# thourihan/DeepfakeDetection

Measured on AMD Instinct MI355X. Metric: train images/sec @224^2 (EfficientNet-B0), higher is better.
Workload: dtype bf16

## Files before the change

deepfakedetection_amd/_lib.py:

```python

from __future__ import annotations

import ctypes
from ctypes import POINTER, Structure, c_double, c_float, c_int, c_int64, c_long, c_size_t, c_uint32, c_void_p
from pathlib import Path

import os as _os

LIB_PATH = Path(_os.environ.get("DFD_LIB_PATH") or Path(__file__).resolve().parent / "libdfd_hip.so")

DFD_OK = 0
ERRORS = {-1: "DFD_EINVAL", -2: "DFD_EUNSUPPORTED", -3: "DFD_ELAUNCH", -4: "DFD_EWORKSPACE"}
F32, BF16 = 0, 1
ACT_NONE, ACT_SILU, ACT_RELU, ACT_GELU = 0, 1, 2, 3
PRO_NONE, PRO_BN_ACT, PRO_BN_ACT_GATE, PRO_AFFINE2 = 0, 1, 2, 3
MAX_PARTIALS = 1024
ADAMW_TABLE_COLS = 5
ADAMW_HP_LEN = 8


class DwShape(Structure):
    _fields_ = [(n, c_int) for n in ("N", "H", "W", "C", "Ho", "Wo", "k", "stride", "pad_top", "pad_left")]


# ... 34 lines not shown
    "dfd_act_bn_bwd_se": (c_int, [c_int, P, P, P, P, P, c_int, P, c_int, c_int, c_int, P, c_int, _PI, P, P, c_int, P, P, P, P, c_int, P]),
    "dfd_prep_weights_multi": (c_int, [P, c_int, P]),
    "dfd_resize_crop_u8": (c_int, [P, P, P, c_int, c_int, c_int, c_int, P]),
    "dfd_augment_u8": (c_int, [P, P, P, c_int, c_int, c_int, P]),
    "dfd_image_prep": (c_int, [P, P, c_int, c_int, c_int, POINTER(c_float), POINTER(c_float), P, P, P]),
    "dfd_pool_ws": (c_size_t, [c_int, c_int, c_int, c_int]),
    "dfd_pool_act": (c_int, [c_int, P, P, c_int, P, c_int, c_int, c_int, P, c_size_t, P]),
    "dfd_pool_bwd_reduce": (c_int, [c_int, P, P, P, c_int, P, c_int, c_int, c_int, P, c_size_t, P]),
    "dfd_scale_rows": (c_int, [c_int, P, P, P, c_int, c_int, c_int, P]),
    "dfd_se_fc_fwd": (c_int, [P, P, P, P, P, c_int, c_int, c_int, c_int, P, P, P, P]),
    "dfd_se_fc_bwd": (c_int, [P, P, P, P, P, P, c_int, c_int, c_int, c_int, P, P, P, P, P, c_int, P, P]),
    "dfd_dwconv_fwd": (c_int, [c_int, P, P, c_int, P, P, POINTER(DwShape), P, c_int, _PI, P]),
    "dfd_dwconv_bwd_data": (c_int, [c_int, P, P, P, P, P, P, c_int, P, POINTER(DwShape), P, c_int, _PI, P]),
    "dfd_dwconv_bwd_weight": (c_int, [c_int, P, P, P, P, P, c_int, P, POINTER(DwShape), c_int, P, c_size_t, P]),
    "dfd_dwconv_bwd_weight_ws": (c_size_t, [POINTER(DwShape)]),
    "dfd_dwconv_bwd_fused": (c_int, [c_int, P, P, P, P, P, P, c_int, P, P, POINTER(DwShape), P, c_int, _PI, c_int, P, c_size_t, P]),
    "dfd_pwconv_fwd": (c_int, [c_int, P, POINTER(Prologue), P, P, P, c_int, c_int, c_int, P, c_int, _PI, P]),
    "dfd_pwconv_wgrad": (c_int, [c_int, P, POINTER(Prologue), c_int, P, POINTER(Prologue), c_int, c_int, P, c_int, P, c_size_t, P]),
    "dfd_pwconv_wgrad_ws": (c_size_t, [c_int, c_int, c_int]),
    "dfd_gradcam_map": (c_int, [P, P, c_int, c_int, c_int, c_int, P, P]),
    "dfd_cam_render": (c_int, [P, c_int, c_int, c_int, c_int, c_int, P, P, P, c_double, P, P, P, c_size_t, P]),
    "dfd_cam_render_ws": (c_size_t, [c_int, c_int, c_int, c_int, c_int]),
    "dfd_pwconv_bwd_fused": (c_int, [c_int, P, P, P, P, P, P, c_int, c_int, c_int, P, P, c_int, P, c_size_t, P]),
    "dfd_pw_prep_weights": (c_int, [c_int, P, P, P, c_int, c_int, P]),
    "dfd_stem_conv_fwd": (c_int, [c_int, P, P, P, POINTER(StemShape), P, c_int, _PI, P]),
    "dfd_stem_conv_wgrad": (c_int, [c_int, P, P, P, P, P, POINTER(StemShape), c_int, P, c_size_t, P]),
    "dfd_stem_conv_wgrad_ws": (c_size_t, [POINTER(StemShape)]),
    "dfd_dropout": (c_int, [P, P, c_float, P, c_int, P]),
    "dfd_linear_fwd": (c_int, [P, P, P, P, c_int, c_int, c_int, P]),
    "dfd_linear_bwd": (c_int, [P, P, P, P, P, P, c_int, c_int, c_int, c_int, P]),
    "dfd_ce_loss": (c_int, [P, P, c_int, c_int, c_float, c_float, P, P, P, P]),
    "dfd_softmax_argmax": (c_int, [P, c_int, c_int, P, P, P]),
    "dfd_adamw_step": (c_int, [P, c_int, P, P]),
    "dfd_bn_eval_coeffs_multi": (c_int, [P, c_int, P]),
    "dfd_sum_batch_begin": (c_int, []),
    "dfd_sum_batch_end": (c_int, []),
    "dfd_sum_batch_end_deferred": (c_int, []),
    "dfd_sum_passengers_flush": (c_int, [P]),
    "dfd_sum_passengers_discard": (c_int, []),
    "dfd_se_fwd": (c_int, [c_int, P, P, c_int, c_int, c_int, c_int, P, P, P, P, c_int, c_int, P, P, P, P, P, c_size_t, P]),
    "dfd_se_bwd": (c_int, [c_int, P, P, P, c_int, c_int, c_int, c_int, P, P, P, P, P, c_int, c_int, P, P, P, P, P, P, c_int,
                           P, c_size_t, P, P]),
    "dfd_pwconv_fwd_eval": (c_int, [c_int, P, P, P, c_int, P, c_int, c_int, c_int, P]),
    "dfd_dwconv_fwd_eval_tiles": (c_int, [c_int, P]),
    "dfd_dwconv_fwd_eval": (c_int, [c_int, P, P, P, c_int, P, P, P, P, P]),
    "dfd_se_fwd_parts": (c_int, [P, c_int, c_int, c_int, c_int, P, P, P, P, c_int, c_int, P, P, P, P, P]),
# ... 122 lines not shown
```

deepfakedetection_amd/csrc/dfd_pwtnw.hip:

```cpp
#include "dfd_pw.h"

#define TNW_MIN_ROWS 16

template <int ROWS, int NA, int NBT, int PA, int PB, int ACT, int DG = 0>
__global__ void __launch_bounds__(DFD_THREADS, NBT > 9 ? 1 : 2)
k_pw_tnw(const bf16* __restrict__ a, ProArgs pa, int Na, const bf16* __restrict__ b, ProArgs pb, int Nb, int M,
         int rows_per_block, int swap, float* __restrict__ ws, const bf16* __restrict__ w_kn = nullptr,
         const bf16* __restrict__ res = nullptr, bf16* __restrict__ dx = nullptr, int wstride = 0, int woff = 0) {
    constexpr int ITA = (ROWS * NA * 2 + 63) / 64;
    constexpr int ITB = (ROWS * NBT * 2 + 63) / 64;
    extern __shared__ __attribute__((aligned(16))) unsigned char smem[];
    const int t = threadIdx.x, lane = t & 63, wave = t >> 6;
    unsigned char* at = smem + wave * (2 * ROWS * 256);
    unsigned char* bt = at + ROWS * 256;
    float* cl = reinterpret_cast<float*>(smem + 4 * 2 * ROWS * 256);
    const bf16* a2 = reinterpret_cast<const bf16*>(pa.a2);
    const bf16* b2 = reinterpret_cast<const bf16*>(pb.a2);
    const int ca = Na >> 3, cb = Nb >> 3;
    float* gc = cl + 3 * (Na + Nb) + wave * 2 * Nb;
    int gimg = -1;

    for (int i = t; i < 3 * Na; i += DFD_THREADS) cl[i] = (PA != DFD_PRO_NONE) ? pa.coef[i] : 0.f;
    for (int i = t; i < 3 * Nb; i += DFD_THREADS) {
        float v = 0.f;
        if (PB == DFD_PRO_AFFINE2) v = pb.coef[i];
        else if (PB != DFD_PRO_NONE && i < 2 * Nb) v = pb.coef[i];
        cl[3 * Na + i] = v;
    }
    for (int i = t; i < 4 * 2 * ROWS * 256 / 16; i += DFD_THREADS) reinterpret_cast<uint4*>(smem)[i] = make_uint4(0, 0, 0, 0);
    if constexpr (DG) {
        const int chunks = wstride >> 4;
        for (int i = t; i < NA * 16 * chunks; i += DFD_THREADS) {
            const int r = i / chunks, c = i - r * chunks;
            uint4 v = make_uint4(0, 0, 0, 0);
            if (r < Na && c < cb) v = *reinterpret_cast<const uint4*>(w_kn + (long)r * Nb + c * 8);
            *reinterpret_cast<uint4*>(smem + woff + r * wstride + c * 16) = v;
        }
    }
    __syncthreads();

    int ra[ITA], cha[ITA], rb[ITB], chb[ITB];
#pragma unroll
    for (int i = 0; i < ITA; ++i) {
        const int idx = lane + 64 * i;
        const bool ok = idx < ROWS * ca;
        ra[i] = ok ? idx / ca : -1;
        cha[i] = ok ? idx - ra[i] * ca : 0;
    }
#pragma unroll
    for (int i = 0; i < ITB; ++i) {
        const int idx = lane + 64 * i;
        const bool ok = idx < ROWS * cb;
        rb[i] = ok ? idx / cb : -1;
        chb[i] = ok ? idx - rb[i] * cb : 0;
    }

    f32x4_t acc[NA][NBT];
#pragma unroll
    for (int x = 0; x < NA; ++x)
#pragma unroll
        for (int y = 0; y < NBT; ++y) acc[x][y] = (f32x4_t){0.f, 0.f, 0.f, 0.f};
    const int na = (Na + 15) >> 4, nbt = (Nb + 15) >> 4;
    constexpr int RT = ROWS / 16;
    f32x4_t accd[DG ? NA : 1][RT];

    const int rows_per_wave = rows_per_block / 4;
    const int mbeg = blockIdx.x * rows_per_block + wave * rows_per_wave;
    int mend = mbeg + rows_per_wave;
    if (mend > M) mend = M;

    uint4 va[ITA], va2[ITA], vb[ITB], vb2[ITB];
    auto load_a = [&](int i, int m0) {
        int row = m0 + (ra[i] < 0 ? 0 : ra[i]);
        row = row < M ? row : M - 1;
        const long off = (long)row * Na + cha[i] * 8;
        va[i] = *reinterpret_cast<const uint4*>(a + off);
        if constexpr (PA == DFD_PRO_AFFINE2) va2[i] = *reinterpret_cast<const uint4*>(a2 + off);
    };
    auto load_b = [&](int i, int m0) {
        int row = m0 + (rb[i] < 0 ? 0 : rb[i]);
        row = row < M ? row : M - 1;
        const long off = (long)row * Nb + chb[i] * 8;
        vb[i] = *reinterpret_cast<const uint4*>(b + off);
        if constexpr (PB == DFD_PRO_AFFINE2) vb2[i] = *reinterpret_cast<const uint4*>(b2 + off);
    };
    auto g_load = [&](int m0) {
#pragma unroll
        for (int i = 0; i < ITA; ++i) load_a(i, m0);
#pragma unroll
        for (int i = 0; i < ITB; ++i) load_b(i, m0);
    };
    auto pro_item = [&](auto mode_tag, uint4 q, uint4 q2, const float* cf, int N, int ch, int m, const ProArgs& pr) -> uint4 {
        constexpr int MODE = decltype(mode_tag)::value;
        if constexpr (MODE == DFD_PRO_NONE) {
            return q;
        } else {
            float v[8], c0[8], c1[8];
            q_to_f(q, v);
            load_f32<8>(cf + ch * 8, c0);
            load_f32<8>(cf + N + ch * 8, c1);
            if constexpr (MODE == DFD_PRO_AFFINE2) {
                float v2[8], c2[8];
                q_to_f(q2, v2);
                load_f32<8>(cf + 2 * N + ch * 8, c2);
#pragma unroll
                for (int j = 0; j < 8; ++j) v[j] = fmaf(c0[j], v[j], fmaf(c1[j], v2[j], c2[j]));
            } else if constexpr (MODE == DFD_PRO_BN_ACT) {
// ... 5 lines not shown
#pragma unroll
                for (int j = 0; j < 8; ++j) v[j] = round_to<bf16>(v[j]) * gt[j];
            }
            return f_to_q(v);
        }
    };
    auto s_store_a = [&](int m0) {
#pragma unroll
        for (int i = 0; i < ITA; ++i) {
            if (ra[i] >= 0) {
                uint4 v = make_uint4(0, 0, 0, 0);
                if (m0 + ra[i] < mend) v = pro_item(std::integral_constant<int, PA>{}, va[i], va2[i], cl, Na, cha[i], m0 + ra[i], pa);
                *reinterpret_cast<uint4*>(at + tn_off_bf16(ra[i], cha[i])) = v;
            }
            load_a(i, m0 + ROWS);
        }
    };
    auto s_store_b = [&](int m0, int grp, auto refill_tag) {
        constexpr bool refill = decltype(refill_tag)::value;
#pragma unroll
        for (int i = 0; i < ITB; ++i) {
            if (rb[i] >= 0 && (chb[i] >> 4) == grp) {
                uint4 v = make_uint4(0, 0, 0, 0);
                if (m0 + rb[i] < mend)
                    v = pro_item(std::integral_constant<int, PB>{}, vb[i], vb2[i], cl + 3 * Na, Nb, chb[i], m0 + rb[i], pb);
                *reinterpret_cast<uint4*>(bt + tn_off_bf16(rb[i], chb[i] & 15)) = v;
            }
            if constexpr (refill) load_b(i, m0 + ROWS);
        }
    };
    auto wave_sync = [&]() {
        __builtin_amdgcn_fence(__ATOMIC_RELEASE, "wavefront");
        __builtin_amdgcn_wave_barrier();
        __builtin_amdgcn_fence(__ATOMIC_ACQUIRE, "wavefront");
    };
    const int g = lane >> 4, li = lane & 15, qrow = li >> 2, pcol = li & 3;
    auto frag = [&](const unsigned char* tile, int ch0) -> short8_t {
        const int ch = ch0 + (pcol >> 1), sub = (pcol & 1) << 3;
        if constexpr (ROWS == 32) {
            const int m_lo = 8 * g + qrow, m_hi = m_lo + 4;
            const short4_t lo = __builtin_amdgcn_ds_read_tr16_b64_v4i16(
                (__attribute__((address_space(3))) short4_t*)(tile + tn_off_bf16(m_lo, ch) + sub));
            const short4_t hi = __builtin_amdgcn_ds_read_tr16_b64_v4i16(
                (__attribute__((address_space(3))) short4_t*)(tile + tn_off_bf16(m_hi, ch) + sub));
            return (short8_t){lo[0], lo[1], lo[2], lo[3], hi[0], hi[1], hi[2], hi[3]};
        } else {
            const short4_t lo = __builtin_amdgcn_ds_read_tr16_b64_v4i16(
                (__attribute__((address_space(3))) short4_t*)(tile + tn_off_bf16(4 * g + qrow, ch) + sub));
            return (short8_t){lo[0], lo[1], lo[2], lo[3], 0, 0, 0, 0};
        }
    };
    auto mma = [&](const short8_t& fx, const short8_t& fy, f32x4_t c) -> f32x4_t {
        if constexpr (ROWS == 32) {
            return __builtin_amdgcn_mfma_f32_16x16x32_bf16(__builtin_bit_cast(bf16x8_t, fx), __builtin_bit_cast(bf16x8_t, fy), c, 0, 0, 0);
        } else {
            const short4_t x4 = (short4_t){fx[0], fx[1], fx[2], fx[3]}, y4 = (short4_t){fy[0], fy[1], fy[2], fy[3]};
            return __builtin_amdgcn_mfma_f32_16x16x16bf16_1k(x4, y4, c, 0, 0, 0);
        }
    };

    constexpr int NGRP = NBT > 8 ? 2 : 1;
    if (mbeg < mend) g_load(mbeg);
    for (int m0 = mbeg; m0 < mend; m0 += ROWS) {
        short8_t fa[NA];
        if constexpr (PB == DFD_PRO_BN_ACT_GATE) {
            const int img0 = pro_image(pb, m0);
            if (img0 != gimg) {
                gimg = img0;
                for (int i = lane; i < 2 * Nb; i += 64) {
                    const int im = img0 + (i >= Nb ? 1 : 0);
                    gc[i] = ((long)im * pb.HW < M) ? pb.gate[(long)im * Nb + (i >= Nb ? i - Nb : i)] : 0.f;
                }
                wave_sync();
            }
        }
        if constexpr (DG) {
#pragma unroll
            for (int x = 0; x < NA; ++x)
#pragma unroll
                for (int j = 0; j < RT; ++j) accd[x][j] = (f32x4_t){0.f, 0.f, 0.f, 0.f};
        }
        s_store_a(m0);
        s_store_b(m0, 0, std::integral_constant<bool, NGRP == 1>{});
        wave_sync();
#pragma unroll
        for (int x = 0; x < NA; ++x)
            if (x < na) fa[x] = frag(at, 2 * x);
#pragma unroll
        for (int grp = 0; grp < NGRP; ++grp) {
            if (grp > 0) {
                wave_sync();
                s_store_b(m0, grp, std::true_type{});
                wave_sync();
            }
#pragma unroll
            for (int y = 0; y < NBT; ++y) {
                if ((y >> 3) != grp || y >= nbt) continue;
                const short8_t fb = frag(bt, 2 * (y & 7));
#pragma unroll
                for (int x = 0; x < NA; ++x)
                    if (x < na)
                        acc[x][y] = mma(fa[x], fb, acc[x][y]);
            }
            if constexpr (DG) {
#pragma unroll
                for (int ks = 0; ks < 4; ++ks) {
                    if (grp * 8 + 2 * ks >= NBT || grp * 8 + 2 * ks >= nbt) continue;
                    const int chl = 4 * ks + g, chg = grp * 16 + chl;
                    uint4 fd[RT];
#pragma unroll
                    for (int j = 0; j < RT; ++j) {
                        fd[j] = *reinterpret_cast<const uint4*>(bt + tn_off_bf16(j * 16 + li, chl));
                        if (chg >= cb) fd[j] = make_uint4(0, 0, 0, 0);
                    }
// ... 86 lines not shown
    hipLaunchKernelGGL((k_pw_tnw<ROWS, NA, NBT, PAV, PBV, ACTV>), dim3(nblocks), dim3(DFD_THREADS), lds, st, (const bf16*)a, pa, \
                       Na, (const bf16*)b, pb, Nb, M, rpb, swap, ws)
    if (mb == DFD_PRO_BN_ACT_GATE) {
        if (act != DFD_ACT_SILU) return DFD_EUNSUPPORTED;
        if (ma == DFD_PRO_AFFINE2) LAUNCH_TNW(DFD_PRO_AFFINE2, DFD_PRO_BN_ACT_GATE, DFD_ACT_SILU);
        else LAUNCH_TNW(DFD_PRO_NONE, DFD_PRO_BN_ACT_GATE, DFD_ACT_SILU);
    } else if (mb == DFD_PRO_BN_ACT) {
        if (ma != DFD_PRO_AFFINE2) return DFD_EUNSUPPORTED;
        if (act == DFD_ACT_GELU) LAUNCH_TNW(DFD_PRO_AFFINE2, DFD_PRO_BN_ACT, DFD_ACT_GELU);
        else if (act == DFD_ACT_SILU) LAUNCH_TNW(DFD_PRO_AFFINE2, DFD_PRO_BN_ACT, DFD_ACT_SILU);
        else return DFD_EUNSUPPORTED;
    } else if (mb == DFD_PRO_AFFINE2) {
        if (ma == DFD_PRO_AFFINE2) return DFD_EUNSUPPORTED;
        LAUNCH_TNW(DFD_PRO_NONE, DFD_PRO_AFFINE2, DFD_ACT_NONE);
    } else {
        if (ma == DFD_PRO_AFFINE2) LAUNCH_TNW(DFD_PRO_AFFINE2, DFD_PRO_NONE, DFD_ACT_NONE);
        else LAUNCH_TNW(DFD_PRO_NONE, DFD_PRO_NONE, DFD_ACT_NONE);
    }
#undef LAUNCH_TNW
    if (hipGetLastError() != hipSuccess) return DFD_ELAUNCH;
    return dfd_launch_sum_partials(ws, nblocks, (long)Na * Nb, dw, accumulate, st);
}

template <int ROWS, int NA, int NBT>
static int tnw_dg_launch(const void* x, int Cin, const void* dz, const dfd_prologue* pro_d, int Cm, const void* w_kn, const void* residual,
                         int M, void* dx, float* dw, int accumulate, float* ws, size_t ws_bytes, hipStream_t st) {
    const ProArgs pa = pro_args(nullptr), pb = pro_args(pro_d);
    int nblocks = NBT > 9 ? 256 : 512;
    int rpb = (M + nblocks - 1) / nblocks;
    rpb = (rpb + 4 * ROWS - 1) / (4 * ROWS) * (4 * ROWS);
    nblocks = (M + rpb - 1) / rpb;
    if ((size_t)(nblocks + nblocks / 32 + 2) * Cin * Cm * 4 > ws_bytes) return DFD_EUNSUPPORTED;
    const int wstride = (Cm + 31) / 32 * 64 + 16;
    int woff = 4 * 2 * ROWS * 256 + 3 * (Cin + Cm) * 4;
    woff = (woff + 15) / 16 * 16;
    const int lds = woff + NA * 16 * wstride;
    if (lds > 80 * 1024) return DFD_EUNSUPPORTED;
    struct TnwDgTag;
    dfd_allow_lds_once<TnwDgTag>(k_pw_tnw<ROWS, NA, NBT, DFD_PRO_NONE, DFD_PRO_AFFINE2, DFD_ACT_NONE, 2>, 80 * 1024);
    dfd_allow_lds_once<TnwDgTag>(k_pw_tnw<ROWS, NA, NBT, DFD_PRO_NONE, DFD_PRO_AFFINE2, DFD_ACT_NONE, 1>, 80 * 1024);
    if (residual)
        hipLaunchKernelGGL((k_pw_tnw<ROWS, NA, NBT, DFD_PRO_NONE, DFD_PRO_AFFINE2, DFD_ACT_NONE, 2>), dim3(nblocks), dim3(DFD_THREADS), lds, st,
                           (const bf16*)x, pa, Cin, (const bf16*)dz, pb, Cm, M, rpb, 1, ws, (const bf16*)w_kn, (const bf16*)residual, (bf16*)dx,
                           wstride, woff);
    else
        hipLaunchKernelGGL((k_pw_tnw<ROWS, NA, NBT, DFD_PRO_NONE, DFD_PRO_AFFINE2, DFD_ACT_NONE, 1>), dim3(nblocks), dim3(DFD_THREADS), lds, st,
                           (const bf16*)x, pa, Cin, (const bf16*)dz, pb, Cm, M, rpb, 1, ws, (const bf16*)w_kn, (const bf16*)nullptr, (bf16*)dx,
                           wstride, woff);
    if (hipGetLastError() != hipSuccess) return DFD_ELAUNCH;
    return dfd_launch_sum_partials(ws, nblocks, (long)Cin * Cm, dw, accumulate, st);
}
extern "C" int dfd_pwconv_bwd_fused(int dtype, const void* dz, const void* y, const float* coef, const void* x, const void* w_kn,
                                    const void* residual, int M, int Cm, int Cin, void* dx, float* dw, int accumulate, float* ws,
                                    size_t ws_bytes, dfd_stream stream) {
    if (!dz || !y || !coef || !x || !w_kn || !dx || !dw || !ws || M < 1 || Cm < 8 || Cin < 8 || Cm % 8 || Cin % 8) return DFD_EINVAL;
    if (dtype != DFD_BF16 || M < 2048 * 32 * 3 || Cin > 48 || Cin > Cm || !(Cm <= 128 || (Cm <= 240 && Cm % 16 == 0))) return DFD_EUNSUPPORTED;
    if (Cin > 32 && Cm <= 144) return DFD_EUNSUPPORTED;
    dfd_prologue pro{};
    pro.mode = DFD_PRO_AFFINE2; pro.act = DFD_ACT_NONE; pro.HW = 1; pro.a2 = y; pro.coef = coef; pro.gate = nullptr;
    hipStream_t st = (hipStream_t)stream;
    if (Cm <= 96) return tnw_dg_launch<32, 2, 6>(x, Cin, dz, &pro, Cm, w_kn, residual, M, dx, dw, accumulate, ws, ws_bytes, st);
    if (Cm <= 144) return tnw_dg_launch<16, 2, 9>(x, Cin, dz, &pro, Cm, w_kn, residual, M, dx, dw, accumulate, ws, ws_bytes, st);
    if (Cm <= 192) return tnw_dg_launch<16, 3, 12>(x, Cin, dz, &pro, Cm, w_kn, residual, M, dx, dw, accumulate, ws, ws_bytes, st);
    return tnw_dg_launch<16, 3, 15>(x, Cin, dz, &pro, Cm, w_kn, residual, M, dx, dw, accumulate, ws, ws_bytes, st);
}

int dfd_pw_tnw(const void* p, const dfd_prologue* pro_p, int Ni, const void* q, const dfd_prologue* pro_q, int Nj, int M,
               float* dw, int accumulate, float* ws, size_t ws_bytes, hipStream_t st) {
    if (M < 2048 * 32 * 3) return DFD_EUNSUPPORTED;
    const int mp = pro_p ? pro_p->mode : DFD_PRO_NONE, mq = pro_q ? pro_q->mode : DFD_PRO_NONE;
    const auto wide_ok = [](int n) { return n <= 128 || (n <= 144 && n % 16 == 0); };
#define TNW_PICK(NARROW, WIDE, ...)                                             \
    do {                                                                       \
        if ((NARROW) <= 32 && (WIDE) <= 96) return tnw_launch<32, 2, 6>(__VA_ARGS__); \
        if ((NARROW) <= 32) return tnw_launch<16, 2, 9>(__VA_ARGS__);               \
        return DFD_EUNSUPPORTED;     \
    } while (0)
    if (Ni <= 48 && wide_ok(Nj) && Ni <= Nj && tnw_pro_ok(mp, mq))
        TNW_PICK(Ni, Nj, p, pro_p, Ni, q, pro_q, Nj, M, 0, dw, accumulate, ws, ws_bytes, st);
    if (Nj <= 48 && wide_ok(Ni) && tnw_pro_ok(mq, mp))
        TNW_PICK(Nj, Ni, q, pro_q, Nj, p, pro_p, Ni, M, 1, dw, accumulate, ws, ws_bytes, st);
#undef TNW_PICK
    return DFD_EUNSUPPORTED;
}
```

deepfakedetection_amd/csrc/dfd_rowpass.hip:

```cpp
#include "dfd_common.h"
#include "dfd_se.h"
#include "dfd_sum.h"

template <typename T, int ACT, bool HAS_RES, bool HAS_RS>
__global__ void __launch_bounds__(DFD_THREADS)
k_bn_act_apply(const T* __restrict__ y, const float* __restrict__ bnstate, const T* __restrict__ res,
               const float* __restrict__ rs, T* __restrict__ out, long total_vec, int CV, int C, long vec_per_img) {
    constexpr int V = Vec<T>::N;
    const long stride = (long)gridDim.x * DFD_THREADS;
    const long first = (long)blockIdx.x * DFD_THREADS + threadIdx.x;
    int cv = (int)(first % CV);
    const int cstep = (int)(stride % CV);
    for (long i = first; i < total_vec; i += stride, cv = cv + cstep >= CV ? cv + cstep - CV : cv + cstep) {
        const int c0 = cv * V;
        float v[V], sc[V], sh[V];
        Vec<T>::load(y + i * V, v);
        load_f32<V>(bnstate + c0, sc);
        load_f32<V>(bnstate + C + c0, sh);
        float r = 1.f;
        if constexpr (HAS_RS) r = rs[i / vec_per_img];
        float q[V];
        if constexpr (HAS_RES) Vec<T>::load(res + i * V, q);
        bn_act_array<ACT, V>(v, sc, sh);
#pragma unroll
// ... 659 lines not shown
}
extern "C" int dfd_bn_eval_coeffs(const float* gamma, const float* beta, const float* running_mean,
                                  const float* running_var, float eps, int C, float* bnstate, dfd_stream stream) {
    return dfd_bn_eval_coeffs_ex(gamma, beta, nullptr, nullptr, running_mean, running_var, eps, C, bnstate, stream);
}
extern "C" int dfd_bn_bwd_finalize_ex(const float* partials, int nparts, int C, double count, const float* gamma,
                                      const float* beta, const float* ls_gamma, const float* bnstate, int train,
                                      float* dgamma, float* dbeta, float* dls, float* dbias, int accumulate, float* coef,
                                      dfd_stream stream) {
    if (!partials || nparts < 1 || C < 1 || count <= 0 || !bnstate || !coef) return DFD_EINVAL;
    if (dls && (!ls_gamma || !beta)) return DFD_EINVAL;
    const int threads = FIN_CH * FIN_LANES, grid = (C + FIN_CH - 1) / FIN_CH;
    hipLaunchKernelGGL(k_bn_bwd_finalize, dim3(grid), dim3(threads), 0, (hipStream_t)stream, partials, nparts, C, count,
                       gamma, beta, ls_gamma, bnstate, train, dgamma, dbeta, dls, dbias, accumulate, coef);
    return DFD_CHECK_LAUNCH();
}
extern "C" int dfd_bn_bwd_finalize(const float* partials, int nparts, int C, double count, const float* gamma,
                                   const float* bnstate, int train, float* dgamma, float* dbeta, int accumulate,
                                   float* coef, dfd_stream stream) {
    return dfd_bn_bwd_finalize_ex(partials, nparts, C, count, gamma, nullptr, nullptr, bnstate, train, dgamma, dbeta, nullptr,
                                  nullptr, accumulate, coef, stream);
}

extern "C" int dfd_version(void) { return 136; }
```

deepfakedetection_amd/functions.py:

```python

from __future__ import annotations

import contextlib
import os
import threading
from dataclasses import dataclass

import torch

from . import kernels as K
from ._lib import ACT_NONE, ACT_SILU
from .arch import ConvGeom
from .arena import grad_dest


@dataclass
class BNRef:

    running_mean: torch.Tensor
    running_var: torch.Tensor
    num_batches_tracked: torch.Tensor | None
    momentum: float
    eps: float
    pre: torch.Tensor | None = None
# ... 116 lines not shown
    bn_dw: BNRef
    bn_project: BNRef
    training: bool
    derived: tuple | None = None
    counters: list | None = None
    grad_enabled: bool = True


class MBConvFunction(torch.autograd.Function):

    @staticmethod
    def forward(ctx, x, w_exp, g_exp, b_exp, w_dw, g_dw, b_dw, se_w1, se_b1, se_w2, se_b2, w_proj, g_proj, b_proj,
                row_scale, cfg: MBConvCtx):
        tr = cfg.training
        N, H, W, Cin = x.shape
        dt = x.dtype
        geom = cfg.dw
        Ho, Wo = geom.out_size(H), geom.out_size(W)
        need_bwd = any(ctx.needs_input_grad)
        if not tr and not (need_bwd and cfg.grad_enabled) and eval_fused_enabled(
                N * H * W * (w_exp.shape[0] if cfg.expand else Cin), dt):
            return MBConvFunction._forward_eval(x, w_exp, g_exp, b_exp, w_dw, g_dw, b_dw, se_w1, se_b1, se_w2, se_b2, w_proj,
                                                g_proj, b_proj, cfg, Ho, Wo)
        if cfg.expand:
            wexp_nk, wexp_kn = cfg.derived[0] if cfg.derived is not None else K.prep_weights(w_exp, dt, True, need_bwd)
            y1, parts, n = K.pwconv(x, None, wexp_nk, None, stats=tr)
            st1 = _bn_state(parts, n, N * H * W, cfg.bn_expand, g_exp, b_exp, tr, cfg.counters)
            y2, parts, n = K.dwconv_fwd(y1, st1, ACT_SILU, w_dw, geom.kernel, geom.stride, geom.pad_lead, geom.pad_lead,
                                        Ho, Wo, stats=tr)
        else:
            wexp_kn, y1, st1 = None, None, None
            y2, parts, n = K.dwconv_fwd(x, None, ACT_NONE, w_dw, geom.kernel, geom.stride, geom.pad_lead, geom.pad_lead,
                                        Ho, Wo, stats=tr)
        st2 = _bn_state(parts, n, N * Ho * Wo, cfg.bn_dw, g_dw, b_dw, tr, cfg.counters)
        w1, w2 = se_w1.reshape(se_w1.shape[0], -1), se_w2.reshape(se_w2.shape[0], -1)
        pooled, hpre, gate, w2t = K.se_fwd(y2, st2, ACT_SILU, w1, se_b1, w2, se_b2, ACT_SILU,
                                           cfg.derived[2] if cfg.derived is not None else None)
        wproj_nk, wproj_kn = cfg.derived[1] if cfg.derived is not None else K.prep_weights(w_proj, dt, True, need_bwd)
        pro = K.pro_bn_act_gate(st2, ACT_SILU, gate, Ho * Wo)
        y3, parts, n = K.pwconv(y2, pro, wproj_nk, None, stats=tr)
        st3 = _bn_state(parts, n, N * Ho * Wo, cfg.bn_project, g_proj, b_proj, tr, cfg.counters)
        out = K.bn_act_apply(y3, st3, ACT_NONE, x if cfg.skip else None, row_scale if cfg.skip else None)
        ctx.cfg = cfg
        ctx.pptr = _ptrs(x, w_exp, g_exp, b_exp, w_dw, g_dw, b_dw, se_w1, se_b1, se_w2, se_b2, w_proj, g_proj, b_proj)
        ctx.in_shape = (N, H, W, Cin)
        ctx.has_rs = cfg.skip and row_scale is not None
        ctx.save_for_backward(x, y1, y2, y3, st1, st2, st3, pooled, hpre, gate, wexp_kn, wproj_kn, w_dw, w1, w2t,
                              g_exp, g_dw, g_proj, row_scale if ctx.has_rs else None)
        return out

    @staticmethod
    def _forward_eval(x, w_exp, g_exp, b_exp, w_dw, g_dw, b_dw, se_w1, se_b1, se_w2, se_b2, w_proj, g_proj, b_proj, cfg, Ho, Wo):
        N, H, W, Cin = x.shape
        dt = x.dtype
        geom = cfg.dw
        a1 = x
        if cfg.expand:
            wexp_nk, _ = cfg.derived[0] if cfg.derived is not None else K.prep_weights(w_exp, dt, True, False)
            st1 = _bn_state(None, 0, N * H * W, cfg.bn_expand, g_exp, b_exp, False, cfg.counters)
            a1 = K.pwconv_eval(x, wexp_nk, st1, ACT_SILU)
        st2 = _bn_state(None, 0, N * Ho * Wo, cfg.bn_dw, g_dw, b_dw, False, cfg.counters)
        a2, pool_parts, _ = K.dwconv_eval(a1, w_dw, st2, ACT_SILU, geom.kernel, geom.stride, geom.pad_lead, geom.pad_lead, Ho, Wo)
        w1, w2 = se_w1.reshape(se_w1.shape[0], -1), se_w2.reshape(se_w2.shape[0], -1)
        _, gate, _ = K.se_fwd_parts(pool_parts, Ho * Wo, w1, se_b1, w2, se_b2, ACT_SILU,
                                    cfg.derived[2] if cfg.derived is not None else None)
        wproj_nk, _ = cfg.derived[1] if cfg.derived is not None else K.prep_weights(w_proj, dt, True, False)
        pro = K.pro_bn_act_gate(K.identity_state(x.device, a2.shape[3]), ACT_NONE, gate, Ho * Wo)
        y3, _, _ = K.pwconv(a2, pro, wproj_nk, None, stats=False)
        st3 = _bn_state(None, 0, N * Ho * Wo, cfg.bn_project, g_proj, b_proj, False, cfg.counters)
        return K.bn_act_apply(y3, st3, ACT_NONE, x if cfg.skip else None, None)

    @staticmethod
    def backward(ctx, g):
        cfg: MBConvCtx = ctx.cfg
        (x, y1, y2, y3, st1, st2, st3, pooled, hpre, gate, wexp_kn, wproj_kn, w_dw, w1, w2t,
         g_exp, g_dw, g_proj, row_scale) = ctx.saved_tensors
        need = ctx.needs_input_grad
        tr = cfg.training
        geom = cfg.dw
        N, H, W, Cin = ctx.in_shape
        _, Ho, Wo, Cmid = y2.shape
        with K.sum_batch():
            return MBConvFunction._backward(ctx, g, cfg, x, y1, y2, y3, st1, st2, st3, pooled, hpre, gate, wexp_kn, wproj_kn,
                                            w_dw, w1, w2t, g_exp, g_dw, g_proj, row_scale, need, tr, geom, N, H, W, Cin, Ho, Wo, Cmid)

    @staticmethod
    def _backward(ctx, g, cfg, x, y1, y2, y3, st1, st2, st3, pooled, hpre, gate, wexp_kn, wproj_kn, w_dw, w1, w2t, g_exp, g_dw,
                  g_proj, row_scale, need, tr, geom, N, H, W, Cin, Ho, Wo, Cmid):
        g = _c(g)
        gb = K.scale_rows(g, row_scale) if ctx.has_rs else g
        parts, n = K.bn_bwd_reduce(gb, y3, st3, None)
        Cout, R = y3.shape[3], w1.shape[0]
        coef3, dg_proj, db_proj = K.bn_bwd_finalize(parts, n, N * Ho * Wo, g_proj, st3, tr, need[12] or need[13],
                                                    _dest(ctx, 12, (Cout,)), _dest(ctx, 13, (Cout,)))
        gm3 = K.affine2_apply(gb, y3, coef3)
        D, _, _ = K.pwconv(gm3, None, wproj_kn, None, stats=False)
        dw_proj = None
        if need[11]:
            pro_q = K.pro_bn_act_gate(st2, ACT_SILU, gate, Ho * Wo)
            with K.side_stream(N * Ho * Wo):
                dw_proj = K.pwconv_wgrad(gm3, None, y2, pro_q, _dest(ctx, 11, (Cout, Cmid))).view(Cout, Cmid, 1, 1)
        want_se = need[7] or need[8] or need[9] or need[10]
        se_outs = (_dest(ctx, 7, (R, Cmid)), _dest(ctx, 8, (R,)), _dest(ctx, 9, (Cmid, R)), _dest(ctx, 10, (Cmid,)))
        se_res = K.se_bwd(D, y2, st2, ACT_SILU, gate, hpre, pooled, w1, w2t, ACT_SILU, want_se, se_outs, defer_wgrad=SE_WGRAD_PASSENGER)
        dpooled, dw1, db1, dw2, db2 = se_res[:5]
        se_job = se_res[5] if SE_WGRAD_PASSENGER else None
        dz2, parts, n = K.act_bn_bwd(D, y2, gate, dpooled, st2, ACT_SILU, se_job=se_job)
        if dw1 is not None:
            dw1, dw2 = dw1.view(dw1.shape[0], -1, 1, 1), dw2.view(dw2.shape[0], -1, 1, 1)
        coef2, dg_dw, db_dw = K.bn_bwd_finalize(parts, n, N * Ho * Wo, g_dw, st2, tr, need[5] or need[6],
                                                _dest(ctx, 5, (Cmid,)), _dest(ctx, 6, (Cmid,)))
        kk = geom.kernel
        dw_dw = dx = dw_exp = dg_exp = db_exp = None
        if cfg.expand:
            fused = need[4] and K.dwconv_bwd_fused_ok(geom.kernel, geom.stride)
            if fused:
                dz1, parts, n, dw_dw = K.dwconv_bwd_fused(dz2, y2, coef2, w_dw, y1, st1, ACT_SILU, geom.kernel, geom.stride,
                                                          geom.pad_lead, geom.pad_lead, _dest(ctx, 4, (Cmid, 1, kk, kk)))
            else:
                dz1, parts, n = K.dwconv_bwd_data(dz2, y2, coef2, w_dw, y1, st1, ACT_SILU, y1.shape, geom.kernel,
                                                  geom.stride, geom.pad_lead, geom.pad_lead)
            coef1, dg_exp, db_exp = K.bn_bwd_finalize(parts, n, N * H * W, g_exp, st1, tr, need[2] or need[3],
                                                      _dest(ctx, 2, (Cmid,)), _dest(ctx, 3, (Cmid,)))
            pro_dy1 = K.pro_affine2(y1, coef1)
            both = K.pwconv_bwd_fused(dz1, y1, coef1, x, wexp_kn, g if cfg.skip else None, _dest(ctx, 1, (Cmid, Cin))) \
                if (need[0] and need[1] and K.pwconv_bwd_fused_ok(dz1, x)) else None
            with K.side_stream(N * Ho * Wo):
                if need[4] and not fused:
                    dw_dw = K.dwconv_bwd_weight(dz2, y2, coef2, y1, st1, ACT_SILU, geom.kernel, geom.stride,
                                                geom.pad_lead, geom.pad_lead, _dest(ctx, 4, (Cmid, 1, kk, kk)))
                if need[1] and both is None:
                    dw_exp = K.pwconv_wgrad(dz1, pro_dy1, x, None, _dest(ctx, 1, (Cmid, Cin))).view(Cmid, Cin, 1, 1)
            if both is not None:
                dx, dw_exp = both[0], both[1].view(Cmid, Cin, 1, 1)
            elif need[0]:
                dx, _, _ = K.pwconv(dz1, pro_dy1, wexp_kn, g if cfg.skip else None, stats=False)
        else:
            if need[4]:
                with K.side_stream(N * Ho * Wo):
                    dw_dw = K.dwconv_bwd_weight(dz2, y2, coef2, x, None, ACT_NONE, geom.kernel, geom.stride,
                                                geom.pad_lead, geom.pad_lead, _dest(ctx, 4, (Cmid, 1, kk, kk)))
            if need[0]:
                dx, _, _ = K.dwconv_bwd_data(dz2, y2, coef2, w_dw, None, None, ACT_NONE, ctx.in_shape, geom.kernel,
                                             geom.stride, geom.pad_lead, geom.pad_lead)
                if cfg.skip:
                    dx = K.add(dx, g)
        K.join_side()
        return (dx, dw_exp, dg_exp, db_exp, dw_dw, dg_dw, db_dw, dw1, db1, dw2, db2, dw_proj, dg_proj, db_proj,
                None, None)
# ... 117 lines not shown
```

deepfakedetection_amd/kernels.py:

```python

from __future__ import annotations

import contextlib
import functools
import ctypes
import threading
import weakref
from dataclasses import dataclass

import os

import torch

from . import _lib
from ._lib import (
    ACT_NONE, ACT_SILU, BF16, F32, MAX_PARTIALS, PRO_AFFINE2, PRO_BN_ACT, PRO_BN_ACT_GATE, PRO_NONE,
    DwShape, Prologue, StemShape, check,
)

_scratch: dict[tuple[int, int, str], torch.Tensor] = {}


def _L():
    return _lib.load()
# ... 926 lines not shown
def pwconv_bwd_fused_ok(dz: torch.Tensor, x: torch.Tensor) -> bool:
    Cm, Cin = dz.shape[-1], x.shape[-1]
    M = dz.numel() // Cm
    if not (_FUSE_EXPAND_BWD and dz.dtype == torch.bfloat16 and M >= 2048 * 32 * 3 and Cin <= Cm and Cin % 8 == 0 and Cm % 8 == 0):
        return False
    if Cin <= 32 and (Cm <= 128 or (Cm <= 144 and Cm % 16 == 0)):
        return True
    return _FUSE_EXPAND_WIDE and Cin <= 48 and 144 < Cm <= 240 and Cm % 16 == 0


def pwconv_bwd_fused(dz: torch.Tensor, y: torch.Tensor, coef: torch.Tensor, x: torch.Tensor, w_kn: torch.Tensor,
                     residual: torch.Tensor | None, out_w: torch.Tensor | None = None):
    if not pwconv_bwd_fused_ok(dz, x):
        return None
    Cm, Cin = dz.shape[-1], x.shape[-1]
    M = dz.numel() // Cm
    nbytes = _L().dfd_pwconv_wgrad_ws(M, Cm, Cin)
    ws = scratch(dz.device, "wgrad_ws", nbytes)
    dx = torch.empty_like(x)
    dw = _dst(None if out_w is None else out_w.view(Cm, Cin), (Cm, Cin), dz.device)
    rc = _L().dfd_pwconv_bwd_fused(_dt(dz), _p(dz), _p(y), _p(coef), _p(x), _p(w_kn), _p(residual), M, Cm, Cin, _p(dx), _p(dw), 0,
                                   _p(ws), ws.numel() * 4, _stream())
    check(rc, "dfd_pwconv_bwd_fused", f"M={M} Cm={Cm} Cin={Cin}")
    return dx, dw


def _stem_shape(x_shape, Cout: int, Ho: int, Wo: int, k: int, stride: int, pt: int, pl: int) -> StemShape:
    N, H, W, _ = x_shape
    return StemShape(N, H, W, Cout, Ho, Wo, k, stride, pt, pl)


def stem_conv_fwd(x: torch.Tensor, w: torch.Tensor, out_dtype: torch.dtype, stride: int, pad_top: int, pad_left: int,
                  Ho: int, Wo: int, stats: bool = True):
    _chk_nhwc(x)
    if x.dtype != torch.float32 or x.shape[3] != 3:
        raise ValueError("stem input must be f32 [N,H,W,3]")
    Cout, k = w.shape[0], w.shape[2]
    y = torch.empty((x.shape[0], Ho, Wo, Cout), dtype=out_dtype, device=x.device)
    shp = _stem_shape(x.shape, Cout, Ho, Wo, k, stride, pad_top, pad_left)
    parts = partials_buf(x.device, Cout) if stats else None
    n = ctypes.c_int(0)
    check(_L().dfd_stem_conv_fwd(_dt(y), _p(x), _p(w), _p(y), ctypes.byref(shp), _p(parts), MAX_PARTIALS,
                                 ctypes.byref(n), _stream()), "dfd_stem_conv_fwd")
    return y, parts, n.value


# ... 568 lines not shown
    return fallback


def _timed(name: str, fn):
    def inner(*args, **kwargs):
        sink = _profile_sink
        if sink is None:
            return fn(*args, **kwargs)
        e0, e1 = torch.cuda.Event(enable_timing=True), torch.cuda.Event(enable_timing=True)
        e0.record()
        out = fn(*args, **kwargs)
        e1.record()
        nbytes = _tensor_bytes(args) + _tensor_bytes(list(kwargs.values())) + _tensor_bytes(out)
        sink.append((name, nbytes, _flops(name, args), e0, e1, _bytes_8d(name, args, nbytes)))
        return out

    inner.__name__ = name
    inner.__doc__ = fn.__doc__
    return inner


for _name in _TIMED:
    globals()[_name] = _timed(_name, globals()[_name])

__all__ = [name for name in dir() if not name.startswith("_")]
```

include/dfd_hip.h:

```cpp
#ifndef DFD_HIP_H
#define DFD_HIP_H

#include <stddef.h>
#include <stdint.h>

#ifdef __cplusplus
extern "C" {
#endif

typedef void* dfd_stream;

#define DFD_OK            0
#define DFD_EINVAL       (-1)
#define DFD_EUNSUPPORTED (-2)
#define DFD_ELAUNCH      (-3)
#define DFD_EWORKSPACE   (-4)

#define DFD_F32   0
#define DFD_BF16  1

#define DFD_ACT_NONE 0
#define DFD_ACT_SILU 1
#define DFD_ACT_RELU 2
#define DFD_ACT_GELU 3
// ... 131 lines not shown
#define DFD_PRO_BN_ACT      1
#define DFD_PRO_BN_ACT_GATE 2
#define DFD_PRO_AFFINE2     3
typedef struct {
    int mode;
    int act;
    int HW;
    int _pad;
    const void* a2;
    const float* coef;
    const float* gate;
} dfd_prologue;

int dfd_pwconv_fwd(int dtype, const void* a, const dfd_prologue* pro, const void* w,
                   void* out, const void* residual, int M, int K, int Nout,
                   float* partials, int pcap, int* nparts, dfd_stream stream);
int dfd_pwconv_wgrad(int dtype, const void* p, const dfd_prologue* pro_p, int Ni,
                     const void* q, const dfd_prologue* pro_q, int Nj, int M,
                     float* dw, int accumulate, float* ws, size_t ws_bytes,
                     dfd_stream stream);
int dfd_pwconv_bwd_fused(int dtype, const void* dz, const void* y, const float* coef, const void* x, const void* w_kn,
                         const void* residual, int M, int Cm, int Cin, void* dx, float* dw, int accumulate, float* ws,
                         size_t ws_bytes, dfd_stream stream);
size_t dfd_pwconv_wgrad_ws(int M, int Ni, int Nj);
int dfd_pw_prep_weights(int dtype, const float* w, void* w_nk, void* w_kn, int N, int K,
                        dfd_stream stream);
typedef struct dfd_prep_job {
    const float* src;
    void* nk;
    void* kn;
    int N, K;
    int dtype;
    int _pad;
} dfd_prep_job;
int dfd_prep_weights_multi(const dfd_prep_job* jobs, int njobs, dfd_stream stream);

typedef struct {
    int N, H, W, Cout, Ho, Wo, k, stride, pad_top, pad_left;
} dfd_stem_shape;
int dfd_stem_conv_fwd(int dtype, const float* x, const float* w, void* y,
                      const dfd_stem_shape* s, float* partials, int pcap, int* nparts,
                      dfd_stream stream);
int dfd_stem_conv_wgrad(int dtype, const float* x, const void* dz, const void* y,
                        const float* coef, float* dw, const dfd_stem_shape* s,
                        int accumulate, float* ws, size_t ws_bytes, dfd_stream stream);
size_t dfd_stem_conv_wgrad_ws(const dfd_stem_shape* s);
// ... 171 lines not shown
```

Before: 20730.

## Recompute expand-conv output in fused backward instead of reloading y1

```diff
diff --git a/deepfakedetection_amd/_lib.py b/deepfakedetection_amd/_lib.py
--- a/deepfakedetection_amd/_lib.py
+++ b/deepfakedetection_amd/_lib.py
@@ -80,6 +80,7 @@
     "dfd_cam_render": (c_int, [P, c_int, c_int, c_int, c_int, c_int, P, P, P, c_double, P, P, P, c_size_t, P]),
     "dfd_cam_render_ws": (c_size_t, [c_int, c_int, c_int, c_int, c_int]),
     "dfd_pwconv_bwd_fused": (c_int, [c_int, P, P, P, P, P, P, c_int, c_int, c_int, P, P, c_int, P, c_size_t, P]),
+    "dfd_pwconv_bwd_fused_xpd": (c_int, [c_int, P, P, P, P, P, P, c_int, c_int, c_int, P, P, c_int, P, c_size_t, P]),
     "dfd_pw_prep_weights": (c_int, [c_int, P, P, P, c_int, c_int, P]),
     "dfd_stem_conv_fwd": (c_int, [c_int, P, P, P, POINTER(StemShape), P, c_int, _PI, P]),
     "dfd_stem_conv_wgrad": (c_int, [c_int, P, P, P, P, P, POINTER(StemShape), c_int, P, c_size_t, P]),
diff --git a/deepfakedetection_amd/csrc/dfd_pwtnw.hip b/deepfakedetection_amd/csrc/dfd_pwtnw.hip
--- a/deepfakedetection_amd/csrc/dfd_pwtnw.hip
+++ b/deepfakedetection_amd/csrc/dfd_pwtnw.hip
@@ -1,12 +1,15 @@
 #include "dfd_pw.h"
+#include "dfd_xpd.h"
 
 #define TNW_MIN_ROWS 16
 
-template <int ROWS, int NA, int NBT, int PA, int PB, int ACT, int DG = 0>
+template <int ROWS, int NA, int NBT, int PA, int PB, int ACT, int DG = 0, bool XR = false>
 __global__ void __launch_bounds__(DFD_THREADS, NBT > 9 ? 1 : 2)
 k_pw_tnw(const bf16* __restrict__ a, ProArgs pa, int Na, const bf16* __restrict__ b, ProArgs pb, int Nb, int M,
          int rows_per_block, int swap, float* __restrict__ ws, const bf16* __restrict__ w_kn = nullptr,
-         const bf16* __restrict__ res = nullptr, bf16* __restrict__ dx = nullptr, int wstride = 0, int woff = 0) {
+         const bf16* __restrict__ res = nullptr, bf16* __restrict__ dx = nullptr, int wstride = 0, int woff = 0,
+         const bf16* __restrict__ w_nk = nullptr, int xoff = 0) {
+    static_assert(!XR || (DG && PA == DFD_PRO_NONE && PB == DFD_PRO_AFFINE2), "expand recompute: the fused expand backward only");
     constexpr int ITA = (ROWS * NA * 2 + 63) / 64;
     constexpr int ITB = (ROWS * NBT * 2 + 63) / 64;
     extern __shared__ __attribute__((aligned(16))) unsigned char smem[];
@@ -36,6 +39,7 @@
             if (r < Na && c < cb) v = *reinterpret_cast<const uint4*>(w_kn + (long)r * Nb + c * 8);
             *reinterpret_cast<uint4*>(smem + woff + r * wstride + c * 16) = v;
         }
+        if constexpr (XR) xpd_stage_w(smem + xoff, w_nk, Nb, Na, (Nb + 15) / 16 * 16, t, DFD_THREADS);
     }
     __syncthreads();
 
@@ -82,7 +86,7 @@
         row = row < M ? row : M - 1;
         const long off = (long)row * Nb + chb[i] * 8;
         vb[i] = *reinterpret_cast<const uint4*>(b + off);
-        if constexpr (PB == DFD_PRO_AFFINE2) vb2[i] = *reinterpret_cast<const uint4*>(b2 + off);
+        if constexpr (PB == DFD_PRO_AFFINE2 && !XR) vb2[i] = *reinterpret_cast<const uint4*>(b2 + off);
     };
     auto g_load = [&](int m0) {
 #pragma unroll
@@ -134,9 +138,14 @@
         for (int i = 0; i < ITB; ++i) {
             if (rb[i] >= 0 && (chb[i] >> 4) == grp) {
                 uint4 v = make_uint4(0, 0, 0, 0);
-                if (m0 + rb[i] < mend)
-                    v = pro_item(std::integral_constant<int, PB>{}, vb[i], vb2[i], cl + 3 * Na, Nb, chb[i], m0 + rb[i], pb);
-                *reinterpret_cast<uint4*>(bt + tn_off_bf16(rb[i], chb[i] & 15)) = v;
+                uint4* slot = reinterpret_cast<uint4*>(bt + tn_off_bf16(rb[i], chb[i] & 15));
+                if (m0 + rb[i] < mend) {
+                    uint4 q2;
+                    if constexpr (XR) q2 = *slot;
+                    else q2 = vb2[i];
+                    v = pro_item(std::integral_constant<int, PB>{}, vb[i], q2, cl + 3 * Na, Nb, chb[i], m0 + rb[i], pb);
+                }
+                *slot = v;
             }
             if constexpr (refill) load_b(i, m0 + ROWS);
         }
@@ -171,6 +180,32 @@
         }
     };
 
+    uint4 fx[XR ? RT : 1];
+    auto xpd_load = [&]() {
+        if constexpr (XR) {
+#pragma unroll
+            for (int j = 0; j < RT; ++j) {
+                fx[j] = *reinterpret_cast<const uint4*>(at + tn_off_bf16(j * 16 + li, g));
+                if (g >= ca) fx[j] = make_uint4(0, 0, 0, 0);
+            }
+        }
+    };
+    auto xpd_store = [&](int grp) {
+        if constexpr (XR) {
+#pragma unroll
+            for (int y = 0; y < NBT; ++y) {
+                if ((y >> 3) != grp || y >= nbt) continue;
+                const uint4 fw = *reinterpret_cast<const uint4*>(smem + xoff + xpd_w_off(y * 16 + li, g));
+#pragma unroll
+                for (int j = 0; j < RT; ++j) {
+                    const f32x4_t r = expand_frag(fw, fx[j]);
+                    *reinterpret_cast<uint2*>(bt + tn_off_bf16(j * 16 + li, 2 * (y & 7) + (g >> 1)) + ((g & 1) << 3)) =
+                        make_uint2(pack_bf2(r[0], r[1]), pack_bf2(r[2], r[3]));
+                }
+            }
+        }
+    };
+
     constexpr int NGRP = NBT > 8 ? 2 : 1;
     if (mbeg < mend) g_load(mbeg);
     for (int m0 = mbeg; m0 < mend; m0 += ROWS) {
@@ -193,6 +228,12 @@
                 for (int j = 0; j < RT; ++j) accd[x][j] = (f32x4_t){0.f, 0.f, 0.f, 0.f};
         }
         s_store_a(m0);
+        if constexpr (XR) {
+            wave_sync();
+            xpd_load();
+            xpd_store(0);
+            wave_sync();
+        }
         s_store_b(m0, 0, std::integral_constant<bool, NGRP == 1>{});
         wave_sync();
 #pragma unroll
@@ -202,6 +243,10 @@
         for (int grp = 0; grp < NGRP; ++grp) {
             if (grp > 0) {
                 wave_sync();
+                if constexpr (XR) {
+                    xpd_store(grp);
+                    wave_sync();
+                }
                 s_store_b(m0, grp, std::true_type{});
                 wave_sync();
             }
@@ -334,9 +379,10 @@
     return dfd_launch_sum_partials(ws, nblocks, (long)Na * Nb, dw, accumulate, st);
 }
 
-template <int ROWS, int NA, int NBT>
+template <int ROWS, int NA, int NBT, bool XR = false>
 static int tnw_dg_launch(const void* x, int Cin, const void* dz, const dfd_prologue* pro_d, int Cm, const void* w_kn, const void* residual,
-                         int M, void* dx, float* dw, int accumulate, float* ws, size_t ws_bytes, hipStream_t st) {
+                         int M, void* dx, float* dw, int accumulate, float* ws, size_t ws_bytes, hipStream_t st,
+                         const void* w_nk = nullptr) {
     const ProArgs pa = pro_args(nullptr), pb = pro_args(pro_d);
     int nblocks = NBT > 9 ? 256 : 512;
     int rpb = (M + nblocks - 1) / nblocks;
@@ -346,19 +392,20 @@
     const int wstride = (Cm + 31) / 32 * 64 + 16;
     int woff = 4 * 2 * ROWS * 256 + 3 * (Cin + Cm) * 4;
     woff = (woff + 15) / 16 * 16;
-    const int lds = woff + NA * 16 * wstride;
+    const int xoff = woff + NA * 16 * wstride;
+    const int lds = xoff + (XR ? (Cm + 15) / 16 * 16 * XPD_ROW_BYTES : 0);
     if (lds > 80 * 1024) return DFD_EUNSUPPORTED;
     struct TnwDgTag;
-    dfd_allow_lds_once<TnwDgTag>(k_pw_tnw<ROWS, NA, NBT, DFD_PRO_NONE, DFD_PRO_AFFINE2, DFD_ACT_NONE, 2>, 80 * 1024);
-    dfd_allow_lds_once<TnwDgTag>(k_pw_tnw<ROWS, NA, NBT, DFD_PRO_NONE, DFD_PRO_AFFINE2, DFD_ACT_NONE, 1>, 80 * 1024);
+    dfd_allow_lds_once<TnwDgTag>(k_pw_tnw<ROWS, NA, NBT, DFD_PRO_NONE, DFD_PRO_AFFINE2, DFD_ACT_NONE, 2, XR>, 80 * 1024);
+    dfd_allow_lds_once<TnwDgTag>(k_pw_tnw<ROWS, NA, NBT, DFD_PRO_NONE, DFD_PRO_AFFINE2, DFD_ACT_NONE, 1, XR>, 80 * 1024);
     if (residual)
-        hipLaunchKernelGGL((k_pw_tnw<ROWS, NA, NBT, DFD_PRO_NONE, DFD_PRO_AFFINE2, DFD_ACT_NONE, 2>), dim3(nblocks), dim3(DFD_THREADS), lds, st,
+        hipLaunchKernelGGL((k_pw_tnw<ROWS, NA, NBT, DFD_PRO_NONE, DFD_PRO_AFFINE2, DFD_ACT_NONE, 2, XR>), dim3(nblocks), dim3(DFD_THREADS), lds, st,
                            (const bf16*)x, pa, Cin, (const bf16*)dz, pb, Cm, M, rpb, 1, ws, (const bf16*)w_kn, (const bf16*)residual, (bf16*)dx,
-                           wstride, woff);
+                           wstride, woff, (const bf16*)w_nk, xoff);
     else
-        hipLaunchKernelGGL((k_pw_tnw<ROWS, NA, NBT, DFD_PRO_NONE, DFD_PRO_AFFINE2, DFD_ACT_NONE, 1>), dim3(nblocks), dim3(DFD_THREADS), lds, st,
+        hipLaunchKernelGGL((k_pw_tnw<ROWS, NA, NBT, DFD_PRO_NONE, DFD_PRO_AFFINE2, DFD_ACT_NONE, 1, XR>), dim3(nblocks), dim3(DFD_THREADS), lds, st,
                            (const bf16*)x, pa, Cin, (const bf16*)dz, pb, Cm, M, rpb, 1, ws, (const bf16*)w_kn, (const bf16*)nullptr, (bf16*)dx,
-                           wstride, woff);
+                           wstride, woff, (const bf16*)w_nk, xoff);
     if (hipGetLastError() != hipSuccess) return DFD_ELAUNCH;
     return dfd_launch_sum_partials(ws, nblocks, (long)Cin * Cm, dw, accumulate, st);
 }
@@ -375,6 +422,19 @@
     if (Cm <= 144) return tnw_dg_launch<16, 2, 9>(x, Cin, dz, &pro, Cm, w_kn, residual, M, dx, dw, accumulate, ws, ws_bytes, st);
     if (Cm <= 192) return tnw_dg_launch<16, 3, 12>(x, Cin, dz, &pro, Cm, w_kn, residual, M, dx, dw, accumulate, ws, ws_bytes, st);
     return tnw_dg_launch<16, 3, 15>(x, Cin, dz, &pro, Cm, w_kn, residual, M, dx, dw, accumulate, ws, ws_bytes, st);
+}
+
+extern "C" int dfd_pwconv_bwd_fused_xpd(int dtype, const void* dz, const float* coef, const void* x, const void* w_nk, const void* w_kn,
+                                        const void* residual, int M, int Cm, int Cin, void* dx, float* dw, int accumulate, float* ws,
+                                        size_t ws_bytes, dfd_stream stream) {
+    if (!dz || !coef || !x || !w_nk || !w_kn || !dx || !dw || !ws || M < 1 || Cm < 8 || Cin < 8 || Cm % 8 || Cin % 8) return DFD_EINVAL;
+    if (dtype != DFD_BF16 || M < 2048 * 32 * 3 || Cin > 32 || Cin > Cm || !(Cm <= 128 || (Cm <= 144 && Cm % 16 == 0)))
+        return DFD_EUNSUPPORTED;
+    dfd_prologue pro{};
+    pro.mode = DFD_PRO_AFFINE2; pro.act = DFD_ACT_NONE; pro.HW = 1; pro.a2 = nullptr; pro.coef = coef; pro.gate = nullptr;
+    hipStream_t st = (hipStream_t)stream;
+    if (Cm <= 96) return tnw_dg_launch<32, 2, 6, true>(x, Cin, dz, &pro, Cm, w_kn, residual, M, dx, dw, accumulate, ws, ws_bytes, st, w_nk);
+    return tnw_dg_launch<16, 2, 9, true>(x, Cin, dz, &pro, Cm, w_kn, residual, M, dx, dw, accumulate, ws, ws_bytes, st, w_nk);
 }
 
 int dfd_pw_tnw(const void* p, const dfd_prologue* pro_p, int Ni, const void* q, const dfd_prologue* pro_q, int Nj, int M,
diff --git a/deepfakedetection_amd/csrc/dfd_rowpass.hip b/deepfakedetection_amd/csrc/dfd_rowpass.hip
--- a/deepfakedetection_amd/csrc/dfd_rowpass.hip
+++ b/deepfakedetection_amd/csrc/dfd_rowpass.hip
@@ -705,4 +705,4 @@
                                   nullptr, accumulate, coef, stream);
 }
 
-extern "C" int dfd_version(void) { return 136; }
+extern "C" int dfd_version(void) { return 137; }
diff --git a/deepfakedetection_amd/csrc/dfd_xpd.h b/deepfakedetection_amd/csrc/dfd_xpd.h
--- /dev/null
+++ b/deepfakedetection_amd/csrc/dfd_xpd.h
@@ -0,0 +1,20 @@
+#pragma once
+#include "dfd_pw.h"
+
+__device__ __forceinline__ f32x4_t expand_frag(uint4 w_frag, uint4 x_frag) {
+    return __builtin_amdgcn_mfma_f32_16x16x32_bf16(__builtin_bit_cast(bf16x8_t, w_frag), __builtin_bit_cast(bf16x8_t, x_frag),
+                                                   (f32x4_t){0.f, 0.f, 0.f, 0.f}, 0, 0, 0);
+}
+
+#define XPD_ROW_BYTES 64
+__device__ __forceinline__ int xpd_w_off(int c, int q) { return c * XPD_ROW_BYTES + ((q ^ ((c >> 2) & 3)) << 4); }
+
+__device__ __forceinline__ void xpd_stage_w(unsigned char* panel, const bf16* __restrict__ w_nk, int Cm, int Cin, int rows, int t,
+                                            int nthreads) {
+    for (int i = t; i < rows * 4; i += nthreads) {
+        const int c = i >> 2, q = i & 3;
+        uint4 v = make_uint4(0, 0, 0, 0);
+        if (c < Cm && q * 8 < Cin) v = *reinterpret_cast<const uint4*>(w_nk + (long)c * Cin + q * 8);
+        *reinterpret_cast<uint4*>(panel + xpd_w_off(c, q)) = v;
+    }
+}
diff --git a/deepfakedetection_amd/functions.py b/deepfakedetection_amd/functions.py
--- a/deepfakedetection_amd/functions.py
+++ b/deepfakedetection_amd/functions.py
@@ -162,6 +162,7 @@
                 N * H * W * (w_exp.shape[0] if cfg.expand else Cin), dt):
             return MBConvFunction._forward_eval(x, w_exp, g_exp, b_exp, w_dw, g_dw, b_dw, se_w1, se_b1, se_w2, se_b2, w_proj,
                                                 g_proj, b_proj, cfg, Ho, Wo)
+        wexp_nk = None
         if cfg.expand:
             wexp_nk, wexp_kn = cfg.derived[0] if cfg.derived is not None else K.prep_weights(w_exp, dt, True, need_bwd)
             y1, parts, n = K.pwconv(x, None, wexp_nk, None, stats=tr)
@@ -185,7 +186,7 @@
         ctx.pptr = _ptrs(x, w_exp, g_exp, b_exp, w_dw, g_dw, b_dw, se_w1, se_b1, se_w2, se_b2, w_proj, g_proj, b_proj)
         ctx.in_shape = (N, H, W, Cin)
         ctx.has_rs = cfg.skip and row_scale is not None
-        ctx.save_for_backward(x, y1, y2, y3, st1, st2, st3, pooled, hpre, gate, wexp_kn, wproj_kn, w_dw, w1, w2t,
+        ctx.save_for_backward(x, y1, y2, y3, st1, st2, st3, pooled, hpre, gate, wexp_nk, wexp_kn, wproj_kn, w_dw, w1, w2t,
                               g_exp, g_dw, g_proj, row_scale if ctx.has_rs else None)
         return out
 
@@ -213,7 +214,7 @@
     @staticmethod
     def backward(ctx, g):
         cfg: MBConvCtx = ctx.cfg
-        (x, y1, y2, y3, st1, st2, st3, pooled, hpre, gate, wexp_kn, wproj_kn, w_dw, w1, w2t,
+        (x, y1, y2, y3, st1, st2, st3, pooled, hpre, gate, wexp_nk, wexp_kn, wproj_kn, w_dw, w1, w2t,
          g_exp, g_dw, g_proj, row_scale) = ctx.saved_tensors
         need = ctx.needs_input_grad
         tr = cfg.training
@@ -221,11 +222,11 @@
         N, H, W, Cin = ctx.in_shape
         _, Ho, Wo, Cmid = y2.shape
         with K.sum_batch():
-            return MBConvFunction._backward(ctx, g, cfg, x, y1, y2, y3, st1, st2, st3, pooled, hpre, gate, wexp_kn, wproj_kn,
+            return MBConvFunction._backward(ctx, g, cfg, x, y1, y2, y3, st1, st2, st3, pooled, hpre, gate, wexp_nk, wexp_kn, wproj_kn,
                                             w_dw, w1, w2t, g_exp, g_dw, g_proj, row_scale, need, tr, geom, N, H, W, Cin, Ho, Wo, Cmid)
 
     @staticmethod
-    def _backward(ctx, g, cfg, x, y1, y2, y3, st1, st2, st3, pooled, hpre, gate, wexp_kn, wproj_kn, w_dw, w1, w2t, g_exp, g_dw,
+    def _backward(ctx, g, cfg, x, y1, y2, y3, st1, st2, st3, pooled, hpre, gate, wexp_nk, wexp_kn, wproj_kn, w_dw, w1, w2t, g_exp, g_dw,
                   g_proj, row_scale, need, tr, geom, N, H, W, Cin, Ho, Wo, Cmid):
         g = _c(g)
         gb = K.scale_rows(g, row_scale) if ctx.has_rs else g
@@ -263,8 +264,11 @@
             coef1, dg_exp, db_exp = K.bn_bwd_finalize(parts, n, N * H * W, g_exp, st1, tr, need[2] or need[3],
                                                       _dest(ctx, 2, (Cmid,)), _dest(ctx, 3, (Cmid,)))
             pro_dy1 = K.pro_affine2(y1, coef1)
-            both = K.pwconv_bwd_fused(dz1, y1, coef1, x, wexp_kn, g if cfg.skip else None, _dest(ctx, 1, (Cmid, Cin))) \
-                if (need[0] and need[1] and K.pwconv_bwd_fused_ok(dz1, x)) else None
+            both = None
+            if need[0] and need[1] and K.pwconv_bwd_fused_ok(dz1, x):
+                res, dst = g if cfg.skip else None, _dest(ctx, 1, (Cmid, Cin))
+                both = K.pwconv_bwd_fused_xpd(dz1, wexp_nk, coef1, x, wexp_kn, res, dst) if K.expand_recompute(dz1, x) \
+                    else K.pwconv_bwd_fused(dz1, y1, coef1, x, wexp_kn, res, dst)
             with K.side_stream(N * Ho * Wo):
                 if need[4] and not fused:
                     dw_dw = K.dwconv_bwd_weight(dz2, y2, coef2, y1, st1, ACT_SILU, geom.kernel, geom.stride,
diff --git a/deepfakedetection_amd/kernels.py b/deepfakedetection_amd/kernels.py
--- a/deepfakedetection_amd/kernels.py
+++ b/deepfakedetection_amd/kernels.py
@@ -972,6 +972,36 @@
     rc = _L().dfd_pwconv_bwd_fused(_dt(dz), _p(dz), _p(y), _p(coef), _p(x), _p(w_kn), _p(residual), M, Cm, Cin, _p(dx), _p(dw), 0,
                                    _p(ws), ws.numel() * 4, _stream())
     check(rc, "dfd_pwconv_bwd_fused", f"M={M} Cm={Cm} Cin={Cin}")
+    return dx, dw
+
+
+_EXPAND_RECOMPUTE = os.environ.get("DFD_EXPAND_RECOMPUTE", "1") != "0"
+_EXPAND_RECOMPUTE_MAX_CM = 96
+
+
+def pwconv_bwd_fused_xpd_ok(dz: torch.Tensor, x: torch.Tensor) -> bool:
+    Cm, Cin = dz.shape[-1], x.shape[-1]
+    return Cin <= 32 and Cm <= 144 and pwconv_bwd_fused_ok(dz, x)
+
+
+def expand_recompute(dz: torch.Tensor, x: torch.Tensor) -> bool:
+    return _EXPAND_RECOMPUTE and dz.shape[-1] <= _EXPAND_RECOMPUTE_MAX_CM and pwconv_bwd_fused_xpd_ok(dz, x)
+
+
+def pwconv_bwd_fused_xpd(dz: torch.Tensor, w_nk: torch.Tensor, coef: torch.Tensor, x: torch.Tensor, w_kn: torch.Tensor,
+                         residual: torch.Tensor | None, out_w: torch.Tensor | None = None):
+    if not pwconv_bwd_fused_xpd_ok(dz, x):
+        return None
+    Cm, Cin = dz.shape[-1], x.shape[-1]
+    M = dz.numel() // Cm
+    assert tuple(w_nk.shape) == (Cm, Cin) and w_nk.dtype == dz.dtype, (tuple(w_nk.shape), w_nk.dtype)
+    nbytes = _L().dfd_pwconv_wgrad_ws(M, Cm, Cin)
+    ws = scratch(dz.device, "wgrad_ws", nbytes)
+    dx = torch.empty_like(x)
+    dw = _dst(None if out_w is None else out_w.view(Cm, Cin), (Cm, Cin), dz.device)
+    rc = _L().dfd_pwconv_bwd_fused_xpd(_dt(dz), _p(dz), _p(coef), _p(x), _p(w_nk), _p(w_kn), _p(residual), M, Cm, Cin, _p(dx), _p(dw),
+                                       0, _p(ws), ws.numel() * 4, _stream())
+    check(rc, "dfd_pwconv_bwd_fused_xpd", f"M={M} Cm={Cm} Cin={Cin}")
     return dx, dw
 
 
@@ -1586,5 +1616,6 @@
 
 for _name in _TIMED:
     globals()[_name] = _timed(_name, globals()[_name])
+pwconv_bwd_fused_xpd = _timed("pwconv_bwd_fused", pwconv_bwd_fused_xpd)
 
 __all__ = [name for name in dir() if not name.startswith("_")]
diff --git a/include/dfd_hip.h b/include/dfd_hip.h
--- a/include/dfd_hip.h
+++ b/include/dfd_hip.h
@@ -177,6 +177,9 @@
 int dfd_pwconv_bwd_fused(int dtype, const void* dz, const void* y, const float* coef, const void* x, const void* w_kn,
                          const void* residual, int M, int Cm, int Cin, void* dx, float* dw, int accumulate, float* ws,
                          size_t ws_bytes, dfd_stream stream);
+int dfd_pwconv_bwd_fused_xpd(int dtype, const void* dz, const float* coef, const void* x, const void* w_nk, const void* w_kn,
+                             const void* residual, int M, int Cm, int Cin, void* dx, float* dw, int accumulate, float* ws,
+                             size_t ws_bytes, dfd_stream stream);
 size_t dfd_pwconv_wgrad_ws(int M, int Ni, int Nj);
 int dfd_pw_prep_weights(int dtype, const float* w, void* w_nk, void* w_kn, int N, int K,
                         dfd_stream stream);
```

After: 20930 (median of 6 runs). No clear change (+1.0%).
